# ANRGUSC/DEFER

Hardware: NVIDIA H100
Metric: inferences_per_sec (higher is better)
Workload: dtype bf16x3->f32

## Files before the change

### defer_b200/csrc/conv_umma.cu

```cuda
#include <cuda.h>
#include <string.h>

#include <type_traits>

#include <vector>

#include "common.cuh"
#include "conv_umma.cuh"

namespace defer {

static int env_int(const char* name, int dflt) {
  const char* v = getenv(name);
  return v ? atoi(v) : dflt;
}

namespace {

constexpr int BM = 128;
constexpr int BK = 64;
constexpr int CONS_THREADS = 256;
constexpr int NUM_THREADS = CONS_THREADS + 128;
constexpr int SMEM_CAP = 227 * 1024 - 256;
constexpr int CTL_BYTES = 256;
constexpr int MAX_STAGES = 8;
constexpr int MEGA_BN = 64;
constexpr int STG_COLS = 64;
constexpr int STG_BYTES = BM * STG_COLS * 4;

struct KParams {
  int n, ho, wo, cout;
  int tile_n, tile_h, tile_w, tiles_h, tiles_w;
  int flat;
  int m_total;
  int kh, kw, sh, sw, pad_t, pad_l;
  int cblocks;
  int k_blocks;
  int splits;
  int cluster;
  uint32_t flags;
  const float* scale;
  const float* shift;
  const void* res;
  void* y;
  float* partial;
  unsigned int* counters;
  size_t plane_out;
};

struct alignas(128) MegaOp {
  CUtensorMap tmx[2];
  CUtensorMap tmw[2];
  KParams p;
  int m_tiles, n_tiles;
  const float* stem_x;
  int stem_h, stem_w, stem_cin, stem_kh, stem_kw, stem_sh, stem_sw, stem_pad_t, stem_pad_l, stem_K;
  int stem_win_rows, stem_win_cols;
  const uint8_t* stem_u8;
  float stem_shift[3];
  const float* scale2;
  const float* shift2;
  void* y2;
  int relu2;
  int store_first;
};

template <int NPLANES, int BN>
struct Smem {
  static constexpr int A_PLANE = BM * 128;
  static constexpr int B_PLANE = BN * 128;
  static constexpr int STAGE = NPLANES * (A_PLANE + B_PLANE);
  static constexpr int RED = BM * BN * 4;
  __host__ __device__ static constexpr int ring(int stages, bool red) {
    return (red && stages * STAGE < RED) ? RED : stages * STAGE;
  }
  __host__ __device__ static constexpr int total(int stages, bool red) {
    return ring(stages, red) + STG_BYTES + CTL_BYTES + 1024;
  }
  __host__ __device__ static constexpr int max_stages() {
    return (SMEM_CAP - STG_BYTES - CTL_BYTES - 1024) / STAGE > MAX_STAGES ? MAX_STAGES
                                                                          : (SMEM_CAP - STG_BYTES - CTL_BYTES - 1024) / STAGE;
  }
};
static_assert(Smem<2, 128>::max_stages() == 3 && Smem<2, 64>::max_stages() == 4, "BF16X2 ring depths");
static_assert(Smem<1, 64>::max_stages() == 8 && Smem<1, 128>::max_stages() == 6, "BF16 ring depths");

__device__ __forceinline__ uint32_t smem_u32(const void* p) { return (uint32_t)__cvta_generic_to_shared(p); }

__device__ __forceinline__ void mbar_init(uint32_t bar, uint32_t count) {
  asm volatile("mbarrier.init.shared::cta.b64 [%0], %1;" ::"r"(bar), "r"(count));
}
__device__ __forceinline__ void mbar_arrive_expect_tx(uint32_t bar, uint32_t bytes) {
  asm volatile("mbarrier.arrive.expect_tx.shared::cta.b64 _, [%0], %1;" ::"r"(bar), "r"(bytes) : "memory");
}
__device__ __forceinline__ void mbar_expect_tx(uint32_t bar, uint32_t bytes) {
  asm volatile("mbarrier.expect_tx.relaxed.cta.shared::cta.b64 [%0], %1;" ::"r"(bar), "r"(bytes) : "memory");
}
__device__ __forceinline__ void mbar_arrive(uint32_t bar) {
  asm volatile("mbarrier.arrive.shared::cta.b64 _, [%0];" ::"r"(bar) : "memory");
}
__device__ __forceinline__ bool mbar_try_wait(uint32_t bar, uint32_t parity) {
  uint32_t ok;
  asm volatile(
      "{\n.reg .pred p;\n"
      "mbarrier.try_wait.parity.shared::cta.b64 p, [%1], %2;\n"
      "selp.u32 %0, 1, 0, p;\n}\n"
      : "=r"(ok)
      : "r"(bar), "r"(parity)
      : "memory");
  return ok != 0;
}
__device__ __forceinline__ unsigned long long gtimer() {
  unsigned long long t;
  asm volatile("mov.u64 %0, %%globaltimer;" : "=l"(t));
  return t;
}
__device__ int g_conv_wait_timeout_tag;
__device__ __forceinline__ void mbar_wait(uint32_t bar, uint32_t parity, int tag) {
  if (mbar_try_wait(bar, parity)) return;
  unsigned long long t0 = gtimer();
  unsigned spins = 0;
  while (!mbar_try_wait(bar, parity)) {
    if ((++spins & 0xfff) == 0 && gtimer() - t0 > 2000000000ull) {
      g_conv_wait_timeout_tag = tag;
      asm volatile("trap;");
    }
  }
}

__device__ __forceinline__ void tma_load_4d(uint32_t dst, const CUtensorMap* map, uint32_t bar, int c0, int c1, int c2,
                                            int c3) {
  asm volatile(
      "cp.async.bulk.tensor.4d.shared::cluster.global.mbarrier::complete_tx::bytes [%0], [%1, {%3, %4, %5, %6}], [%2];"
      ::"r"(dst), "l"(reinterpret_cast<uint64_t>(map)), "r"(bar), "r"(c0), "r"(c1), "r"(c2), "r"(c3)
      : "memory");
}
__device__ __forceinline__ void tma_load_3d(uint32_t dst, const CUtensorMap* map, uint32_t bar, int c0, int c1, int c2) {
  asm volatile(
      "cp.async.bulk.tensor.3d.shared::cluster.global.mbarrier::complete_tx::bytes [%0], [%1, {%3, %4, %5}], [%2];"
      ::"r"(dst), "l"(reinterpret_cast<uint64_t>(map)), "r"(bar), "r"(c0), "r"(c1), "r"(c2)
      : "memory");
}

__device__ __forceinline__ void cluster_sync_all() {
  asm volatile("barrier.cluster.arrive.release.aligned;" ::: "memory");
  asm volatile("barrier.cluster.wait.acquire.aligned;" ::: "memory");
}
__device__ __forceinline__ uint32_t cluster_ctarank() {
  uint32_t r;
  asm volatile("mov.u32 %0, %%cluster_ctarank;" : "=r"(r));
  return r;
}
__device__ __forceinline__ uint32_t cluster_nctarank() {
  uint32_t r;
  asm volatile("mov.u32 %0, %%cluster_nctarank;" : "=r"(r));
  return r;
}
__device__ __forceinline__ uint32_t dsmem_map(uint32_t local_addr, uint32_t rank) {
  uint32_t r;
  asm volatile("mapa.shared::cluster.u32 %0, %1, %2;" : "=r"(r) : "r"(local_addr), "r"(rank));
  return r;
}
__device__ __forceinline__ float4 dsmem_ld4(uint32_t addr) {
  float4 v;
  asm volatile("ld.shared::cluster.v4.f32 {%0, %1, %2, %3}, [%4];" : "=f"(v.x), "=f"(v.y), "=f"(v.z), "=f"(v.w) : "r"(addr));
  return v;
}
__device__ __forceinline__ void cons_bar_sync() { asm volatile("bar.sync 1, 256;" ::: "memory"); }
__device__ __forceinline__ void prod_bar_sync() { asm volatile("bar.sync 2, 128;" ::: "memory"); }

__device__ __forceinline__ uint64_t make_sw128_desc(uint32_t smem_addr) {
  return (uint64_t)((smem_addr & 0x3FFFF) >> 4) | (1ull << 16) | (64ull << 32) | (1ull << 62);
}
__device__ __forceinline__ void wg_fence() { asm volatile("wgmma.fence.sync.aligned;" ::: "memory"); }
__device__ __forceinline__ void wg_commit() { asm volatile("wgmma.commit_group.sync.aligned;" ::: "memory"); }
template <int N>
__device__ __forceinline__ void wg_wait() {
  asm volatile("wgmma.wait_group.sync.aligned %0;" ::"n"(N) : "memory");
}
template <int R>
__device__ __forceinline__ void acc_fence(float (&d)[R]) {
#pragma unroll
  for (int i = 0; i < R; ++i) asm volatile("" : "+f"(d[i])::"memory");
}

template <int BN>
__device__ __forceinline__ void wgmma_bf16(float (&d)[BN / 2], uint64_t a, uint64_t b);
// ... 244 lines not shown
  __shared__ int s_is_last;

  const int tid = threadIdx.x;
  if (tid == 0) {
    for (int s = 0; s < stages; ++s) {
      mbar_init(full_bar(s), 1);
      mbar_init(empty_bar(s), CONS_THREADS / 32);
    }
    asm volatile("fence.mbarrier_init.release.cluster;" ::: "memory");
  }
  __syncthreads();
  if (pdl) {
    asm volatile("griddepcontrol.wait;" ::: "memory");
    asm volatile("griddepcontrol.launch_dependents;" ::: "memory");
  }

  uint32_t it = 0;
  for (int o = 0; o < n_ops; ++o) {
    const MegaOp& op = ops[o];
    const KParams& p = op.p;
    const int total = op.m_tiles * op.n_tiles;
    int t_first, t_step;
    if (MODE == 0) {
      t_first = blockIdx.y * op.m_tiles + blockIdx.x;
      t_step = total;
    } else if (MODE == 1) {
      t_first = blockIdx.x;
      t_step = gridDim.x;
    } else {
      t_first = (int)cluster_ctarank();
      t_step = (int)cluster_nctarank();
    }
    const int split = MODE == 0 ? (int)blockIdx.z : 0;
    const int kb_begin = (split * p.k_blocks) / p.splits;
    const int kb_end = ((split + 1) * p.k_blocks) / p.splits;

    for (int t = t_first; t < total; t += t_step) {
      const int m_tile = t % op.m_tiles;
      const int c_base = (t / op.m_tiles) * BN;
      int n0 = 0, h0 = 0, w0 = 0;
      if (p.flat) {
        w0 = m_tile * BM;
      } else {
        const int tw = m_tile % p.tiles_w;
        const int t2 = m_tile / p.tiles_w;
        n0 = (t2 / p.tiles_h) * p.tile_n;
        h0 = (t2 % p.tiles_h) * p.tile_h;
        w0 = tw * p.tile_w;
      }

      if (tid >= CONS_THREADS) {
        if (tid == CONS_THREADS) {
          const uint32_t a_rows = p.flat ? (uint32_t)BM : (uint32_t)(p.tile_n * p.tile_h * p.tile_w);
          uint32_t i2 = it;
          for (int kb = kb_begin; kb < kb_end; ++kb, ++i2) {
            const int stage = (int)(i2 % (uint32_t)stages);
            const uint32_t phase = (i2 / (uint32_t)stages) & 1u;
            mbar_wait(empty_bar(stage), phase ^ 1u, 1);
            const uint32_t a_dst = ring + stage * L::STAGE;
            const uint32_t b_dst = a_dst + NPLANES * L::A_PLANE;
            const int tap = kb / p.cblocks;
            const int cb = kb - tap * p.cblocks;
            const int khi = tap / p.kw;
            const int kwi = tap - khi * p.kw;
            int cw = w0, ch = 0, cn = 0;
            if (!p.flat) {
              cw = w0 * p.sw + kwi - p.pad_l;
              ch = h0 * p.sh + khi - p.pad_t;
              cn = n0;
            }
            mbar_arrive_expect_tx(full_bar(stage), NPLANES * (a_rows * 128u + (uint32_t)L::B_PLANE));
            tma_load_4d(a_dst, &op.tmx[0], full_bar(stage), cb * BK, cw, ch, cn);
            tma_load_3d(b_dst, &op.tmw[0], full_bar(stage), cb * BK, c_base, tap);
            if (NPLANES == 2) {
              tma_load_4d(a_dst + L::A_PLANE, &op.tmx[1], full_bar(stage), cb * BK, cw, ch, cn);
              tma_load_3d(b_dst + L::B_PLANE, &op.tmw[1], full_bar(stage), cb * BK, c_base, tap);
            }
          }
        }
        it += (uint32_t)(kb_end - kb_begin);
        continue;
      }

      const int wg = tid >> 7;
      const int lane = tid & 31;
      float acc[R];
#pragma unroll
      for (int i = 0; i < R; ++i) acc[i] = 0.f;
      int prev_stage = -1;
      for (int kb = kb_begin; kb < kb_end; ++kb, ++it) {
        const int stage = (int)(it % (uint32_t)stages);
        mbar_wait(full_bar(stage), (it / (uint32_t)stages) & 1u, 2);
        const uint32_t a_addr = ring + stage * L::STAGE + wg * (64 * 128);
        const uint32_t b_addr = ring + stage * L::STAGE + NPLANES * L::A_PLANE;
        wg_fence();
#pragma unroll
        for (int k = 0; k < BK / 16; ++k) {
          const uint64_t a_hi = make_sw128_desc(a_addr + k * 32);
          const uint64_t b_hi = make_sw128_desc(b_addr + k * 32);
          wgmma_bf16<BN>(acc, a_hi, b_hi);
          if (NPLANES == 2) {
            wgmma_bf16<BN>(acc, make_sw128_desc(a_addr + L::A_PLANE + k * 32), b_hi);
            wgmma_bf16<BN>(acc, a_hi, make_sw128_desc(b_addr + L::B_PLANE + k * 32));
          }
        }
        wg_commit();
        wg_wait<1>();
        acc_fence(acc);
        if (prev_stage >= 0 && lane == 0) mbar_arrive(empty_bar(prev_stage));
        prev_stage = stage;
      }
      wg_wait<0>();
      acc_fence(acc);
      if (prev_stage >= 0 && lane == 0) mbar_arrive(empty_bar(prev_stage));


      if (MODE == 0 && p.cluster) {
        cons_bar_sync();
        float4* red_buf = reinterpret_cast<float4*>(smem);
#pragma unroll
        for (int q = 0; q < R / 4; ++q)
          red_buf[q * CONS_THREADS + tid] = make_float4(acc[4 * q], acc[4 * q + 1], acc[4 * q + 2], acc[4 * q + 3]);
        break;
      }
      if (MODE == 0 && p.splits > 1) {
        const size_t tile_lin = (size_t)t;
        float4* mine = reinterpret_cast<float4*>(p.partial) + (tile_lin * p.splits + split) * (R / 4) * CONS_THREADS;
#pragma unroll
        for (int q = 0; q < R / 4; ++q)
// ... 313 lines not shown
          wgmma_bf16<64>(acc, make_sw128_desc(a_addr + L::A_PLANE + k * 32), b_hi);
          wgmma_bf16<64>(acc, a_hi, make_sw128_desc(b_addr + L::B_PLANE + k * 32));
        }
      }
      wg_commit();
      wg_wait<1>();
      acc_fence(acc);
      if (prev_stage >= 0 && lane == 0) mbar_arrive(empty_bar(prev_stage));
      prev_stage = stage;
    }
    wg_wait<0>();
    acc_fence(acc);
    if (prev_stage >= 0 && lane == 0) mbar_arrive(empty_bar(prev_stage));
    int n0, h0, w0;
    stem_tile_origin(p, t % op.m_tiles, n0, h0, w0);
    epi_tile<NPLANES, 64, false>(p, epi_args(op), stg, acc, 0xffffu, (t / op.m_tiles) * 64, n0, h0, w0);
  }
}

template <int NPLANES>
__global__ void __launch_bounds__(NUM_THREADS, 1) conv_stem_kernel(const MegaOp* __restrict__ ops, int stages, int pdl) {
  stem_body<NPLANES, STEM_F32>(ops, stages, pdl);
}

template <int NPLANES>
__global__ void __launch_bounds__(NUM_THREADS, 1) conv_stem_u8_kernel(const MegaOp* __restrict__ ops, int stages, int pdl) {
  stem_body<NPLANES, STEM_U8_CAFFE>(ops, stages, pdl);
}

template <int NPLANES>
__global__ void __launch_bounds__(NUM_THREADS, 1) conv_stem_u8tf_kernel(const MegaOp* __restrict__ ops, int stages, int pdl) {
  stem_body<NPLANES, STEM_U8_TF>(ops, stages, pdl);
}

__global__ void __launch_bounds__(256) weight_transform_kernel(const float* __restrict__ w, __nv_bfloat16* __restrict__ out,
                                                               int taps, int cin, int cout, int nplanes) {
  size_t total = (size_t)taps * cin * cout;
  size_t i = (size_t)blockIdx.x * blockDim.x + threadIdx.x;
  if (i >= total) return;
  int ci = (int)(i % cin);
  size_t t2 = i / cin;
  int co = (int)(t2 % cout);
  int tap = (int)(t2 / cout);
  float v = w[((size_t)tap * cin + ci) * cout + co];
  __nv_bfloat16 hi = __float2bfloat16_rn(v);
  out[i] = hi;
  if (nplanes == 2) out[total + i] = __float2bfloat16_rn(v - __bfloat162float(hi));
}

typedef CUresult (*PFN_encodeTiled)(CUtensorMap*, CUtensorMapDataType, cuuint32_t, void*, const cuuint64_t*,
                                    const cuuint64_t*, const cuuint32_t*, const cuuint32_t*, CUtensorMapInterleave,
                                    CUtensorMapSwizzle, CUtensorMapL2promotion, CUtensorMapFloatOOBfill);

PFN_encodeTiled get_encode() {
  static PFN_encodeTiled fn = nullptr;
  if (!fn) {
    void* p = nullptr;
    cudaDriverEntryPointQueryResult q;
    if (cudaGetDriverEntryPoint("cuTensorMapEncodeTiled", &p, cudaEnableDefault, &q) == cudaSuccess &&
        q == cudaDriverEntryPointSuccess)
      fn = (PFN_encodeTiled)p;
  }
  return fn;
}

int encode_map(CUtensorMap* map, void* base, int rank, const uint64_t* dims, const uint64_t* strides_bytes,
               const uint32_t* box, const uint32_t* estr) {
  PFN_encodeTiled enc = get_encode();
  if (!enc) {
    set_error("cuTensorMapEncodeTiled entry point not available");
    return DEFER_ERR_CUDA;
  }
  CUresult r = enc(map, CU_TENSOR_MAP_DATA_TYPE_BFLOAT16, (cuuint32_t)rank, base, (const cuuint64_t*)dims,
                   (const cuuint64_t*)strides_bytes, (const cuuint32_t*)box, (const cuuint32_t*)estr,
                   CU_TENSOR_MAP_INTERLEAVE_NONE, CU_TENSOR_MAP_SWIZZLE_128B, CU_TENSOR_MAP_L2_PROMOTION_L2_256B,
                   CU_TENSOR_MAP_FLOAT_OOB_FILL_NONE);
  if (r != CUDA_SUCCESS) {
    set_error("cuTensorMapEncodeTiled failed (CUresult %d): rank %d dims [%llu,%llu,%llu,%llu] box [%u,%u,%u,%u]", (int)r,
              rank, (unsigned long long)dims[0], (unsigned long long)dims[1], (unsigned long long)(rank > 2 ? dims[2] : 0),
              (unsigned long long)(rank > 3 ? dims[3] : 0), box[0], box[1], rank > 2 ? box[2] : 0, rank > 3 ? box[3] : 0);
    return DEFER_ERR_CUDA;
  }
  return DEFER_OK;
}

template <auto kernel>
int set_smem_attr(bool cluster16 = false) {
  static bool attr_set[64] = {false};
  int dev = 0;
  DEFER_CUDA(cudaGetDevice(&dev));
  if (dev < 64 && !attr_set[dev]) {
    DEFER_CUDA(cudaFuncSetAttribute(kernel, cudaFuncAttributeMaxDynamicSharedMemorySize, SMEM_CAP));
    if (cluster16) DEFER_CUDA(cudaFuncSetAttribute(kernel, cudaFuncAttributeNonPortableClusterSizeAllowed, 1));
    prefer_max_smem(kernel);
    attr_set[dev] = true;
  }
  return DEFER_OK;
}

int sm_count() {
  static int sms[64] = {0};
  int dev = 0;
  if (cudaGetDevice(&dev) != cudaSuccess || dev >= 64) return 1;
  if (!sms[dev]) cudaDeviceGetAttribute(&sms[dev], cudaDevAttrMultiProcessorCount, dev);
  return sms[dev] > 0 ? sms[dev] : 1;
}

void fill_op(const UmmaConvPlan& P, const UmmaConvLaneArgs& a, MegaOp* out) {
  MegaOp& op = *out;
  memset(&op, 0, sizeof op);
  op.tmx[0] = a.tmap_x[0];
  op.tmx[1] = a.tmap_x[1];
  op.tmw[0] = P.tmap_w[0];
  op.tmw[1] = P.tmap_w[1];
  KParams& kp = op.p;
  kp.n = P.n; kp.ho = P.ho; kp.wo = P.wo; kp.cout = P.cout;
  kp.tile_n = P.tile_n; kp.tile_h = P.tile_h; kp.tile_w = P.tile_w; kp.tiles_h = P.tiles_h; kp.tiles_w = P.tiles_w;
  kp.flat = P.flat;
  kp.m_total = P.n * P.ho * P.wo;
  kp.kh = P.kh; kp.kw = P.kw; kp.sh = P.sh; kp.sw = P.sw; kp.pad_t = P.pad_t; kp.pad_l = P.pad_l;
  kp.cblocks = P.cin / 64;
  kp.k_blocks = P.k_blocks;
  kp.splits = P.splits;
  kp.cluster = P.cluster;
  kp.flags = P.flags;
  kp.scale = P.scale; kp.shift = P.shift;
  kp.res = (P.flags & DEFER_FLAG_RESIDUAL) ? a.res : nullptr;
  kp.y = a.y;
  kp.partial = a.partial;
  kp.counters = a.counters;
  kp.plane_out = (size_t)P.n * P.ho * P.wo * P.cout;
  op.m_tiles = P.tiles_n * P.tiles_h * P.tiles_w;
  op.n_tiles = P.cout / P.bn;
  op.scale2 = P.scale2;
  op.shift2 = P.shift2;
  op.y2 = a.y2;
  op.relu2 = P.relu2;
  op.store_first = P.aff ? P.store_first : 1;
}

template <int NPLANES, int BN, bool AFF = false>
int launch_op_t(const UmmaConvPlan& P, const UmmaConvLaneArgs& a, cudaStream_t st) {
  using L = Smem<NPLANES, BN>;
  constexpr auto kernel = AFF ? &conv_umma_aff_kernel<NPLANES, BN> : &conv_umma_kernel<NPLANES, BN>;
  DEFER_TRY((set_smem_attr<kernel>()));
  MegaOp op;
  fill_op(P, a, &op);
  int stages = P.stages < 2 ? 2 : (P.stages > L::max_stages() ? L::max_stages() : P.stages);
  const size_t smem = (size_t)L::total(stages, P.cluster != 0);
  dim3 grid(op.m_tiles, op.n_tiles, P.splits);
  static const int pdl = env_int("DEFER_PDL", 0);
  if (pdl || P.cluster) {
    cudaLaunchConfig_t cfg;
    memset(&cfg, 0, sizeof cfg);
    cfg.gridDim = grid;
    cfg.blockDim = dim3(NUM_THREADS, 1, 1);
    cfg.dynamicSmemBytes = smem;
    cfg.stream = st;
    cudaLaunchAttribute attr[2];
    int na = 0;
    if (pdl) {
      attr[na].id = cudaLaunchAttributeProgrammaticStreamSerialization;
      attr[na].val.programmaticStreamSerializationAllowed = 1;
      ++na;
    }
    if (P.cluster) {
      attr[na].id = cudaLaunchAttributeClusterDimension;
      attr[na].val.clusterDim.x = 1;
      attr[na].val.clusterDim.y = 1;
      attr[na].val.clusterDim.z = (unsigned)P.splits;
      ++na;
    }
    cfg.attrs = attr;
    cfg.numAttrs = na;
    DEFER_CUDA(cudaLaunchKernelEx(&cfg, kernel, op, stages, pdl));
    return DEFER_OK;
  }
  kernel<<<grid, NUM_THREADS, smem, st>>>(op, stages, 0);
  DEFER_CUDA(cudaGetLastError());
  return DEFER_OK;
}

template <auto kernel>
int launch_grid(const void* dev_op, int n_tiles, int stages, size_t smem, cudaStream_t st) {
  DEFER_TRY((set_smem_attr<kernel>()));
  const int sms = sm_count();
  int grid = sms < n_tiles ? sms : n_tiles;
  const int rounds = (n_tiles + grid - 1) / grid;
  grid = (n_tiles + rounds - 1) / rounds;
  static const int pdl = env_int("DEFER_PDL", 0);
  if (pdl) {
    cudaLaunchConfig_t cfg;
    memset(&cfg, 0, sizeof cfg);
    cfg.gridDim = dim3(grid, 1, 1);
    cfg.blockDim = dim3(NUM_THREADS, 1, 1);
    cfg.dynamicSmemBytes = smem;
    cfg.stream = st;
    cudaLaunchAttribute attr[1];
    attr[0].id = cudaLaunchAttributeProgrammaticStreamSerialization;
    attr[0].val.programmaticStreamSerializationAllowed = 1;
    cfg.attrs = attr;
    cfg.numAttrs = 1;
    DEFER_CUDA(cudaLaunchKernelEx(&cfg, kernel, reinterpret_cast<const MegaOp*>(dev_op), stages, 1));
    return DEFER_OK;
  }
  kernel<<<grid, NUM_THREADS, smem, st>>>(reinterpret_cast<const MegaOp*>(dev_op), stages, 0);
  DEFER_CUDA(cudaGetLastError());
  return DEFER_OK;
}

template <int NPLANES, int BN, bool AFF = false>
int launch_persist_t(const void* dev_op, int n_tiles, int stages, cudaStream_t st) {
  using L = Smem<NPLANES, BN>;
  constexpr auto kernel = AFF ? &conv_stream_aff_kernel<NPLANES, BN> : &conv_stream_kernel<NPLANES, BN>;
  if (stages > L::max_stages()) stages = L::max_stages();
  if (stages < 2) stages = 2;
  return launch_grid<kernel>(dev_op, n_tiles, stages, (size_t)L::total(stages, false), st);
}

template <int NPLANES, int IN>
int launch_stem_t(const void* dev_op, int n_tiles, int stages, cudaStream_t st) {
  using L = StemSmem<NPLANES>;
  constexpr auto kernel = IN == STEM_U8_TF      ? &conv_stem_u8tf_kernel<NPLANES>
                          : IN == STEM_U8_CAFFE ? &conv_stem_u8_kernel<NPLANES>
                                                : &conv_stem_kernel<NPLANES>;
  if (stages > L::max_stages()) stages = L::max_stages();
  if (stages < 2) stages = 2;
  return launch_grid<kernel>(dev_op, n_tiles, stages, (size_t)L::total(stages), st);
}

template <int NPLANES>
int launch_mega_t(const void* dev_ops, int n_ops, int stages, cudaStream_t st) {
  using L = Smem<NPLANES, MEGA_BN>;
  DEFER_TRY(set_smem_attr<conv_mega_kernel<NPLANES>>(true));
  if (stages < 2) stages = 2;
  if (stages > L::max_stages()) stages = L::max_stages();
  const int cluster = umma_mega_cluster_size();
  cudaLaunchConfig_t cfg;
  memset(&cfg, 0, sizeof cfg);
  cfg.gridDim = dim3(cluster, 1, 1);
  cfg.blockDim = dim3(NUM_THREADS, 1, 1);
  cfg.dynamicSmemBytes = L::total(stages, false);
  cfg.stream = st;
  cudaLaunchAttribute attr[1];
  attr[0].id = cudaLaunchAttributeClusterDimension;
  attr[0].val.clusterDim.x = cluster;
  attr[0].val.clusterDim.y = 1;
  attr[0].val.clusterDim.z = 1;
  cfg.attrs = attr;
  cfg.numAttrs = 1;
  DEFER_CUDA(cudaLaunchKernelEx(&cfg, conv_mega_kernel<NPLANES>, reinterpret_cast<const MegaOp*>(dev_ops), n_ops, stages));
  return DEFER_OK;
}

}

bool umma_conv_supported(int fmt, int n, int h, int w, int cin, int ho, int wo, int cout, int kh, int kw, int sh, int sw,
                         int pad_t, int pad_l) {
  if (fmt != FMT_BF16X2 && fmt != FMT_BF16) return false;
  if (cin % 64 != 0 || cout % 64 != 0) return false;
  if (sh < 1 || sw < 1 || sh > 2 || sw > 2) return false;
  if (kh > 7 || kw > 7) return false;
  if (n < 1 || ho < 1 || wo < 1 || h < 1 || w < 1) return false;
  if ((size_t)n * ho * wo * cout >= (1ull << 40)) return false;
  (void)pad_t; (void)pad_l;
  return true;
}

int umma_conv_prepare(UmmaConvPlan* plan, int fmt, int n, int h, int w, int cin, int ho, int wo, int cout, int kh, int kw,
                      int sh, int sw, int pad_t, int pad_l, uint32_t flags, const float* w_hwio_dev, const float* scale_dev,
                      const float* shift_dev, bool mega, int stream_bn) {
  UmmaConvPlan& P = *plan;
  P = UmmaConvPlan();
  P.fmt = fmt;
  P.nplanes = fmt == FMT_BF16X2 ? 2 : 1;
  P.n = n; P.h = h; P.w = w; P.cin = cin; P.ho = ho; P.wo = wo; P.cout = cout;
  P.kh = kh; P.kw = kw; P.sh = sh; P.sw = sw; P.pad_t = pad_t; P.pad_l = pad_l;
  P.flags = flags;
  P.scale = scale_dev;
  P.shift = shift_dev;
  const int taps = kh * kw;
  P.k_blocks = taps * (cin / 64);

  P.flat = (kh == 1 && kw == 1 && sh == 1 && sw == 1 && pad_t == 0 && pad_l == 0 && ho == h && wo == w) ? 1 : 0;
  if (P.flat) {
    long long m = (long long)n * ho * wo;
    P.tile_n = 1; P.tile_h = 1; P.tile_w = BM;
    P.tiles_n = 1; P.tiles_h = 1; P.tiles_w = (int)((m + BM - 1) / BM);
  } else {
    int parts_w = (wo + BM - 1) / BM;
    P.tile_w = (wo + parts_w - 1) / parts_w;
    P.tiles_w = (wo + P.tile_w - 1) / P.tile_w;
    P.tile_h = BM / P.tile_w;
    if (P.tile_h > ho) P.tile_h = ho;
    P.tiles_h = (ho + P.tile_h - 1) / P.tile_h;
    P.tile_h = (ho + P.tiles_h - 1) / P.tiles_h;
    P.tile_n = 1;
    if (P.tile_h == ho && P.tiles_w == 1) {
      P.tile_n = BM / (P.tile_h * P.tile_w);
      if (P.tile_n > n) P.tile_n = n;
      if (P.tile_n < 1) P.tile_n = 1;
    }
    P.tiles_n = (n + P.tile_n - 1) / P.tile_n;
    if (P.tile_w * sw > 256 || P.tile_h * sh > 256) {
      set_error("umma conv: TMA box too large (tile %dx%d stride %dx%d)", P.tile_h, P.tile_w, sh, sw);
      return DEFER_ERR_INVALID;
    }
  }
  const int m_tiles = P.tiles_n * P.tiles_h * P.tiles_w;

  P.bn = (cout % 128 == 0 && (long long)m_tiles * (cout / 128) >= env_int("DEFER_UMMA_BN128_MIN_CTAS", 1)) ? 128 : 64;
  int force_bn = env_int("DEFER_UMMA_BN", 0);
  if (force_bn == 64 || (force_bn == 128 && cout % 128 == 0)) P.bn = force_bn;
  int ctas = m_tiles * (cout / P.bn);
  P.splits = 1;
  int target = env_int("DEFER_UMMA_TARGET_CTAS", 4);
  if (env_int("DEFER_UMMA_SPLITK", 1) && ctas < target && P.k_blocks >= 8) {
    int s = (target + ctas - 1) / ctas;
    int max_s = P.k_blocks / 4;
    if (s > max_s) s = max_s;
    if (s > 16) s = 16;
    if (s < 1) s = 1;
    int per = (P.k_blocks + s - 1) / s;
    P.splits = (P.k_blocks + per - 1) / per;
  }
  int force_split = env_int("DEFER_UMMA_FORCE_SPLITS", 0);
  if (force_split > 0 && force_split <= P.k_blocks) {
    int per = (P.k_blocks + force_split - 1) / force_split;
    P.splits = (P.k_blocks + per - 1) / per;
  }
  P.cluster = 0;
  if (env_int("DEFER_UMMA_CLUSTER", 0) && force_split <= 0 && !mega) {
    const int min_kb = env_int("DEFER_UMMA_CSPLIT_KB", 4);
    int max_s = env_int("DEFER_UMMA_CSPLIT_MAX", 8);
    if (max_s > 8) max_s = 8;
    const int max_ctas = env_int("DEFER_UMMA_CSPLIT_MAX_CTAS", 256);
    int s = 1;
    for (int c = 2; c <= max_s; c *= 2)
      if (P.k_blocks / c >= min_kb && (long long)ctas * c <= max_ctas) s = c;
    int force_c = env_int("DEFER_UMMA_FORCE_CSPLIT", 0);
    if ((force_c == 2 || force_c == 4 || force_c == 8) && P.k_blocks >= force_c) s = force_c;
    P.splits = s;
    P.cluster = s > 1 ? 1 : 0;
  }
  if (mega) {
    P.bn = MEGA_BN;
    P.splits = 1;
    P.cluster = 0;
  }
  if (stream_bn > 0) {
    P.bn = (stream_bn == 128 && cout % 128 == 0) ? 128 : 64;
    P.splits = 1;
    P.cluster = 0;
    P.stream = 1;
  }
  {
    int kb_per = (P.k_blocks + P.splits - 1) / P.splits;
    int st = kb_per <= 2 ? 2 : (kb_per <= 6 ? 3 : 4);
    int force_st = env_int("DEFER_UMMA_STAGES", 0);
    if (force_st > 0) st = force_st;
    P.stages = st;
  }

  size_t welems = (size_t)taps * cin * cout;
  DEFER_CUDA(cudaMalloc(&P.w_dev, welems * 2 * P.nplanes));
  {
    unsigned grid = (unsigned)((welems + 255) / 256);
    prefer_max_smem(weight_transform_kernel);
    weight_transform_kernel<<<grid, 256>>>(w_hwio_dev, (__nv_bfloat16*)P.w_dev, taps, cin, cout, P.nplanes);
    DEFER_CUDA(cudaGetLastError());
  }
  for (int pl = 0; pl < P.nplanes; ++pl) {
    uint64_t dims[3] = {(uint64_t)cin, (uint64_t)cout, (uint64_t)taps};
    uint64_t strides[2] = {(uint64_t)cin * 2, (uint64_t)cin * cout * 2};
    uint32_t box[3] = {64, (uint32_t)P.bn, 1};
    uint32_t es[3] = {1, 1, 1};
    DEFER_TRY(encode_map(&P.tmap_w[pl], (uint8_t*)P.w_dev + pl * welems * 2, 3, dims, strides, box, es));
  }
  if (P.nplanes == 1) P.tmap_w[1] = P.tmap_w[0];
  P.ready = true;
  return DEFER_OK;
}

int umma_conv_bind(const UmmaConvPlan& P, UmmaConvLaneArgs* a, const void* x, const void* res, void* y) {
  if (!P.ready) {
    set_error("umma_conv_bind: plan not prepared");
    return DEFER_ERR_STATE;
  }
  size_t xelems = (size_t)P.n * P.h * P.w * P.cin;
  for (int pl = 0; pl < P.nplanes; ++pl) {
    uint8_t* base = (uint8_t*)x + pl * xelems * 2;
    if (P.flat) {
      uint64_t m = (uint64_t)P.n * P.h * P.w;
      uint64_t dims[4] = {(uint64_t)P.cin, m, 1, 1};
      uint64_t strides[3] = {(uint64_t)P.cin * 2, m * P.cin * 2, m * P.cin * 2};
      uint32_t box[4] = {64, BM, 1, 1};
      uint32_t es[4] = {1, 1, 1, 1};
      DEFER_TRY(encode_map(&a->tmap_x[pl], base, 4, dims, strides, box, es));
    } else {
      uint64_t dims[4] = {(uint64_t)P.cin, (uint64_t)P.w, (uint64_t)P.h, (uint64_t)P.n};
      uint64_t strides[3] = {(uint64_t)P.cin * 2, (uint64_t)P.w * P.cin * 2, (uint64_t)P.h * P.w * P.cin * 2};
      uint32_t box[4] = {64, (uint32_t)(P.tile_w * P.sw), (uint32_t)(P.tile_h * P.sh), (uint32_t)P.tile_n};
      uint32_t es[4] = {1, (uint32_t)P.sw, (uint32_t)P.sh, 1};
      DEFER_TRY(encode_map(&a->tmap_x[pl], base, 4, dims, strides, box, es));
    }
  }
  if (P.nplanes == 1) a->tmap_x[1] = a->tmap_x[0];
  a->res = res;
  a->y = y;
  a->partial = nullptr;
  a->counters = nullptr;
  if (P.splits > 1 && !P.cluster) {
    size_t tiles = (size_t)P.tiles_n * P.tiles_h * P.tiles_w * (P.cout / P.bn);
    DEFER_CUDA(cudaMalloc((void**)&a->partial, tiles * P.splits * BM * P.bn * sizeof(float)));
    DEFER_CUDA(cudaMalloc((void**)&a->counters, tiles * sizeof(unsigned int)));
    DEFER_CUDA(cudaMemset(a->counters, 0, tiles * sizeof(unsigned int)));
  }
  return DEFER_OK;
}

void umma_conv_unbind(UmmaConvLaneArgs* a) {
  if (a->partial) cudaFree(a->partial);
  if (a->counters) cudaFree(a->counters);
  a->partial = nullptr;
  a->counters = nullptr;
}

int launch_conv_umma(const UmmaConvPlan& P, const UmmaConvLaneArgs& a, cudaStream_t st) {
  if (P.aff) {
    if (P.nplanes == 2) return P.bn == 128 ? launch_op_t<2, 128, true>(P, a, st) : launch_op_t<2, 64, true>(P, a, st);
    return P.bn == 128 ? launch_op_t<1, 128, true>(P, a, st) : launch_op_t<1, 64, true>(P, a, st);
  }
  if (P.nplanes == 2) return P.bn == 128 ? launch_op_t<2, 128>(P, a, st) : launch_op_t<2, 64>(P, a, st);
  return P.bn == 128 ? launch_op_t<1, 128>(P, a, st) : launch_op_t<1, 64>(P, a, st);
}

size_t umma_mega_op_bytes() { return sizeof(MegaOp); }

int umma_mega_fill(void* host_dst, const UmmaConvPlan& P, const UmmaConvLaneArgs& a) {
  if (!P.ready || (P.bn != MEGA_BN && !P.stream) || P.splits != 1) {
    set_error("umma_mega_fill: plan is not a persistent-kernel plan (bn %d, splits %d)", P.bn, P.splits);
    return DEFER_ERR_STATE;
  }
  MegaOp op;
  fill_op(P, a, &op);
// ... 102 lines not shown
```

### defer_b200/csrc/conv_umma.cuh

```cuda
#pragma once
#include <cuda.h>
#include <cuda_runtime.h>
#include <stdint.h>

namespace defer {

struct UmmaConvPlan {
  int fmt = 0, nplanes = 1;
  int n = 0, h = 0, w = 0, cin = 0, ho = 0, wo = 0, cout = 0;
  int kh = 1, kw = 1, sh = 1, sw = 1, pad_t = 0, pad_l = 0;
  uint32_t flags = 0;
  int tile_n = 1, tile_h = 1, tile_w = 1, tiles_n = 1, tiles_h = 1, tiles_w = 1;
  int flat = 0;
  int bn = 64;
  int k_blocks = 0;
  int splits = 1;
  int cluster = 0;
  int stages = 4;
  int stream = 0;
  void* w_dev = nullptr;
  const float* scale = nullptr;
  const float* shift = nullptr;
  bool aff = false;
  const float* scale2 = nullptr;
  const float* shift2 = nullptr;
  int relu2 = 0;
  int store_first = 1;
  CUtensorMap tmap_w[2];
  bool ready = false;
};

struct UmmaConvLaneArgs {
  CUtensorMap tmap_x[2];
  bool direct_out = false;
  const void* res = nullptr;
  void* y = nullptr;
  void* y2 = nullptr;
  float* partial = nullptr;
  unsigned int* counters = nullptr;
};

bool umma_conv_supported(int fmt, int n, int h, int w, int cin, int ho, int wo, int cout, int kh, int kw, int sh, int sw,
                         int pad_t, int pad_l);
int umma_conv_prepare(UmmaConvPlan* plan, int fmt, int n, int h, int w, int cin, int ho, int wo, int cout, int kh, int kw,
                      int sh, int sw, int pad_t, int pad_l, uint32_t flags, const float* w_hwio_dev, const float* scale_dev,
                      const float* shift_dev, bool mega = false, int stream_bn = 0);
int umma_conv_bind(const UmmaConvPlan& plan, UmmaConvLaneArgs* args, const void* x, const void* res, void* y);
void umma_conv_unbind(UmmaConvLaneArgs* args);
int launch_conv_umma(const UmmaConvPlan& plan, const UmmaConvLaneArgs& args, cudaStream_t st);
void umma_conv_release(UmmaConvPlan& plan);

size_t umma_mega_op_bytes();
int umma_mega_fill(void* host_dst, const UmmaConvPlan& plan, const UmmaConvLaneArgs& args);
int umma_mega_cluster_size();
int launch_conv_mega(int nplanes, const void* dev_ops, int n_ops, cudaStream_t st);
int launch_conv_stream(int nplanes, int bn, const void* dev_op, int n_tiles, int k_blocks, bool aff, cudaStream_t st);
bool umma_stem_fusable(int fmt, int cin, int ho, int wo, int cout, int kh, int kw, int sh, int sw, uint32_t flags);
int umma_mega_set_stem(void* host_op, const float* x, int h, int w, int cin, int kh, int kw, int sh, int sw, int pad_t, int pad_l);
void umma_mega_set_stem_u8(void* host_op, const uint8_t* x, const float shift[3]);
int launch_conv_stem(int nplanes, const void* dev_op, int n_tiles, bool u8, bool tf, cudaStream_t st);
int launch_conv_persistent(int nplanes, const void* dev_op, int n_tiles, bool aff, cudaStream_t st);

}
```

### defer_b200/csrc/stage.cu

```cuda
#include <stdarg.h>
#include <string.h>
#include <unistd.h>

#include <mutex>
#include <set>
#include <utility>
#include <stdlib.h>
#include <string>
#include <vector>

#include "common.cuh"
#include "conv_umma.cuh"

namespace defer {

static thread_local char g_err[1024] = "";
void set_error(const char* fmt, ...) {
  va_list ap;
  va_start(ap, fmt);
  vsnprintf(g_err, sizeof(g_err), fmt, ap);
  va_end(ap);
}
const char* get_error() { return g_err; }

// ... 641 lines not shown
        return fail(DEFER_ERR_CUDA);
      }
    }
    if (cfg->is_last) {
      if (cudaMallocHost((void**)&L.out_host, s->bufs[cfg->output_buf].elems * 4) != cudaSuccess ||
          cudaMallocHost((void**)&L.status_host, sizeof(int)) != cudaSuccess) {
        set_error("cudaMallocHost result buffer failed");
        return fail(DEFER_ERR_CUDA);
      }
      *L.status_host = 0;
    }
    L.umma.resize(n_ops);
  }
  if (cudaDeviceSynchronize() != cudaSuccess) {
    set_error("device sync after stage setup failed: %s", cudaGetErrorString(cudaGetLastError()));
    return fail(DEFER_ERR_CUDA);
  }
  *out = s;
  return DEFER_OK;
}

int defer_stage_destroy(defer_stage_t s) {
  if (!s) return DEFER_OK;
  cudaSetDevice(s->cfg.device);
  cudaDeviceSynchronize();
  for (auto& L : s->lanes) {
    if (L.exec) cudaGraphExecDestroy(L.exec);
    if (L.graph) cudaGraphDestroy(L.graph);
    if (L.stream) cudaStreamDestroy(L.stream);
    if (L.done) cudaEventDestroy(L.done);
    if (L.join) cudaEventDestroy(L.join);
    if (L.t0) cudaEventDestroy(L.t0);
    if (L.t1) cudaEventDestroy(L.t1);
    for (auto& ua : L.umma) umma_conv_unbind(&ua);
    if (L.out_host) cudaFreeHost(L.out_host);
    if (L.status_host) cudaFreeHost(L.status_host);
  }
  for (auto& op : s->ops)
    if (op.backend == 2 || op.backend == 4) umma_conv_release(op.umma);
  for (void* p : s->workspace) cudaFree(p);
  for (void* p : s->d_weights) if (p) cudaFree(p);
  for (void* p : s->d_weights_bf16) if (p) cudaFree(p);
  if (s->cons_arena && s->cons_is_ipc) cudaIpcCloseMemHandle(s->cons_arena);
  if (s->prod_arena && s->prod_is_ipc) cudaIpcCloseMemHandle(s->prod_arena);
  for (auto& m : s->marks) if (m.ev) cudaEventDestroy(m.ev);
  if (s->job_t0) cudaEventDestroy(s->job_t0);
  if (s->job_t1) cudaEventDestroy(s->job_t1);
  if (s->flush_buf) cudaFree(s->flush_buf);
  if (s->arena) cudaFree(s->arena);
  delete s;
  return DEFER_OK;
}

int defer_stage_describe(defer_stage_t s, char* buf, size_t buf_len) {
  DEFER_CHECK(s && buf && buf_len > 0, "describe: null");
  std::string o;
  char line[512];
  static const char* fm[] = {"f32", "bf16x2", "bf16"};
  snprintf(line, sizeof line, "stage device=%d fmt=%s batch=%d depth=%d first=%d last=%d ops=%zu prod=%d cons=%d\n",
           s->cfg.device, fm[s->cfg.fmt], s->cfg.batch, s->cfg.depth, s->cfg.is_first, s->cfg.is_last, s->ops.size(),
           (int)s->has_prod, (int)s->has_cons);
  o += line;
  for (size_t i = 0; i < s->ops.size(); ++i) {
    const OpRt& op = s->ops[i];
    const Buf& bi = s->bufs[op.d.in0];
    const Buf& bo = s->bufs[op.d.out];
    if (!s->op_group.empty() && s->op_group[i] >= 0 && (int)i == s->groups[s->op_group[i]].first) {
      snprintf(line, sizeof line, "  -- megakernel group: ops %d..%d in one cluster launch --\n", s->groups[s->op_group[i]].first,
               s->groups[s->op_group[i]].last);
      o += line;
    }
    snprintf(line, sizeof line, "  [%2zu] %-22s in b%-3d(%d,%d,%d) res b%-3d -> b%-3d(%d,%d,%d) k=%dx%d s=%d flags=%u  %.3f MB %.3f GF\n", i,
             op.kname.c_str(), op.d.in0, bi.h, bi.w, bi.c, op.d.in1, op.d.out, bo.h, bo.w, bo.c, op.d.kh, op.d.kw, op.d.sh,
             op.d.flags, op.alg_bytes / 1e6, op.alg_flops / 1e9);
    o += line;
    if ((op.backend == 2 || op.backend == 4) && op.umma.ready) {
      const UmmaConvPlan& u = op.umma;
      snprintf(line, sizeof line, "       wgmma tiles: m=%d x n=%d (BN %d) x k-splits %d%s, %d k-blocks, ring %d -> %d CTAs\n",
               u.tiles_n * u.tiles_h * u.tiles_w, u.cout / u.bn, u.bn, u.splits, u.cluster ? " (cluster, DSMEM reduce)" : "",
               u.k_blocks, u.stages, u.tiles_n * u.tiles_h * u.tiles_w * (u.cout / u.bn) * u.splits);
      o += line;
    }
  }
  strncpy(buf, o.c_str(), buf_len - 1);
  buf[buf_len - 1] = 0;
  return DEFER_OK;
}

int defer_stage_io_bytes(defer_stage_t s, uint64_t* in_bytes, uint64_t* out_bytes) {
  DEFER_CHECK(s, "io_bytes: null");
  if (in_bytes) *in_bytes = s->bufs[s->cfg.input_buf].bytes;
  if (out_bytes) *out_bytes = s->bufs[s->cfg.output_buf].bytes;
  return DEFER_OK;
}

static int fill_token(defer_stage_t s, int role, LinkToken* t) {
  memset(t, 0, sizeof(*t));
  t->magic = TOKEN_MAGIC;
  t->role = role;
  t->device = s->cfg.device;
  t->pid = (int)getpid();
  t->depth = s->cfg.depth;
  t->fmt = s->cfg.fmt;
  t->batch = s->cfg.batch;
  t->slot_bytes = role == 0 ? s->bufs[s->cfg.input_buf].bytes : s->bufs[s->cfg.output_buf].bytes;
  t->arena_bytes = s->arena_bytes;
  t->off_slots = CTRL_BYTES;
  t->slot_stride = s->slot_stride;
  t->local_base = (uint64_t)(uintptr_t)s->arena;
  return DEFER_OK;
}

static int apply_token(defer_stage_t s, int role, const LinkToken* t, uint8_t* mapped, bool is_ipc) {
  DEFER_CHECK(t->depth == s->cfg.depth && t->fmt == s->cfg.fmt && t->batch == s->cfg.batch,
              "link: depth/fmt/batch mismatch (peer %d/%d/%d, mine %d/%d/%d)", t->depth, t->fmt, t->batch, s->cfg.depth,
              s->cfg.fmt, s->cfg.batch);
  if (role == 0) {
    DEFER_CHECK(!s->cfg.is_last, "link: the last stage has no consumer");
    DEFER_CHECK(t->slot_bytes == s->bufs[s->cfg.output_buf].bytes, "link: my output is %zu bytes, consumer slot is %llu",
                s->bufs[s->cfg.output_buf].bytes, (unsigned long long)t->slot_bytes);
    s->cons_arena = mapped;
    s->cons_is_ipc = is_ipc;
    s->cons_off_slots = t->off_slots;
    s->cons_slot_stride = t->slot_stride;
    for (int l = 0; l < s->cfg.depth; ++l) {
      void* slot = mapped + t->off_slots + t->slot_stride * l;
      if (s->hop == HOP_COPY) s->lanes[l].peer_out = slot;
      else s->lanes[l].buf[s->cfg.output_buf] = slot;
    }
    s->has_cons = true;
  } else {
    DEFER_CHECK(!s->cfg.is_first, "link: the first stage has no producer");
    DEFER_CHECK(t->slot_bytes == s->bufs[s->cfg.input_buf].bytes, "link: my input is %zu bytes, producer sends %llu",
// ... 586 lines not shown
```

Baseline: 14390.

## Load conv A tiles with TMA im2col mode for flat 128-row M tiling

Adds a TMA im2col tensor map path so non-1x1 convolutions can tile M as contiguous 128 output pixels (flat) instead of 4-D spatial boxes, with per-tap kernel offsets passed to the im2col copy. It is enabled by default when the padding corners fit the 8-bit offset range. The aim is full 128-row tiles with no waste from spatial boxes that do not align with the output shape. It also factors out the persistent grid computation and extends the describe output.

After: 15280 (median of 6 runs). +6.2%, better.

```diff
diff --git a/defer_b200/csrc/conv_umma.cu b/defer_b200/csrc/conv_umma.cu
--- a/defer_b200/csrc/conv_umma.cu
+++ b/defer_b200/csrc/conv_umma.cu
@@ -32,6 +32,7 @@
   int n, ho, wo, cout;
   int tile_n, tile_h, tile_w, tiles_h, tiles_w;
   int flat;
+  int im2col;
   int m_total;
   int kh, kw, sh, sw, pad_t, pad_l;
   int cblocks;
@@ -133,6 +134,14 @@
   asm volatile(
       "cp.async.bulk.tensor.4d.shared::cluster.global.mbarrier::complete_tx::bytes [%0], [%1, {%3, %4, %5, %6}], [%2];"
       ::"r"(dst), "l"(reinterpret_cast<uint64_t>(map)), "r"(bar), "r"(c0), "r"(c1), "r"(c2), "r"(c3)
+      : "memory");
+}
+__device__ __forceinline__ void tma_load_im2col_4d(uint32_t dst, const CUtensorMap* map, uint32_t bar, int c0, int c1, int c2,
+                                                   int c3, uint16_t ow, uint16_t oh) {
+  asm volatile(
+      "cp.async.bulk.tensor.4d.shared::cluster.global.im2col.mbarrier::complete_tx::bytes [%0], [%1, {%3, %4, %5, %6}], [%2], "
+      "{%7, %8};"
+      ::"r"(dst), "l"(reinterpret_cast<uint64_t>(map)), "r"(bar), "r"(c0), "r"(c1), "r"(c2), "r"(c3), "h"(ow), "h"(oh)
       : "memory");
 }
 __device__ __forceinline__ void tma_load_3d(uint32_t dst, const CUtensorMap* map, uint32_t bar, int c0, int c1, int c2) {
@@ -483,6 +492,14 @@
       if (tid >= CONS_THREADS) {
         if (tid == CONS_THREADS) {
           const uint32_t a_rows = p.flat ? (uint32_t)BM : (uint32_t)(p.tile_n * p.tile_h * p.tile_w);
+          int iw = 0, ih = 0, in_ = 0;
+          if (p.im2col) {
+            const int hw = p.ho * p.wo;
+            in_ = w0 / hw;
+            const int oh = (w0 - in_ * hw) / p.wo;
+            ih = oh * p.sh - p.pad_t;
+            iw = (w0 - in_ * hw - oh * p.wo) * p.sw - p.pad_l;
+          }
           uint32_t i2 = it;
           for (int kb = kb_begin; kb < kb_end; ++kb, ++i2) {
             const int stage = (int)(i2 % (uint32_t)stages);
@@ -501,11 +518,14 @@
               cn = n0;
             }
             mbar_arrive_expect_tx(full_bar(stage), NPLANES * (a_rows * 128u + (uint32_t)L::B_PLANE));
-            tma_load_4d(a_dst, &op.tmx[0], full_bar(stage), cb * BK, cw, ch, cn);
-            tma_load_3d(b_dst, &op.tmw[0], full_bar(stage), cb * BK, c_base, tap);
-            if (NPLANES == 2) {
-              tma_load_4d(a_dst + L::A_PLANE, &op.tmx[1], full_bar(stage), cb * BK, cw, ch, cn);
-              tma_load_3d(b_dst + L::B_PLANE, &op.tmw[1], full_bar(stage), cb * BK, c_base, tap);
+#pragma unroll
+            for (int pl = 0; pl < NPLANES; ++pl) {
+              if (p.im2col)
+                tma_load_im2col_4d(a_dst + pl * L::A_PLANE, &op.tmx[pl], full_bar(stage), cb * BK, iw, ih, in_, (uint16_t)kwi,
+                                   (uint16_t)khi);
+              else
+                tma_load_4d(a_dst + pl * L::A_PLANE, &op.tmx[pl], full_bar(stage), cb * BK, cw, ch, cn);
+              tma_load_3d(b_dst + pl * L::B_PLANE, &op.tmw[pl], full_bar(stage), cb * BK, c_base, tap);
             }
           }
         }
@@ -925,15 +945,27 @@
                                     const cuuint64_t*, const cuuint32_t*, const cuuint32_t*, CUtensorMapInterleave,
                                     CUtensorMapSwizzle, CUtensorMapL2promotion, CUtensorMapFloatOOBfill);
 
+typedef CUresult (*PFN_encodeIm2col)(CUtensorMap*, CUtensorMapDataType, cuuint32_t, void*, const cuuint64_t*,
+                                     const cuuint64_t*, const int*, const int*, cuuint32_t, cuuint32_t, const cuuint32_t*,
+                                     CUtensorMapInterleave, CUtensorMapSwizzle, CUtensorMapL2promotion,
+                                     CUtensorMapFloatOOBfill);
+
+void* driver_entry(const char* name) {
+  void* p = nullptr;
+  cudaDriverEntryPointQueryResult q;
+  if (cudaGetDriverEntryPoint(name, &p, cudaEnableDefault, &q) == cudaSuccess && q == cudaDriverEntryPointSuccess) return p;
+  return nullptr;
+}
+
 PFN_encodeTiled get_encode() {
   static PFN_encodeTiled fn = nullptr;
-  if (!fn) {
-    void* p = nullptr;
-    cudaDriverEntryPointQueryResult q;
-    if (cudaGetDriverEntryPoint("cuTensorMapEncodeTiled", &p, cudaEnableDefault, &q) == cudaSuccess &&
-        q == cudaDriverEntryPointSuccess)
-      fn = (PFN_encodeTiled)p;
-  }
+  if (!fn) fn = (PFN_encodeTiled)driver_entry("cuTensorMapEncodeTiled");
+  return fn;
+}
+
+PFN_encodeIm2col get_encode_im2col() {
+  static PFN_encodeIm2col fn = nullptr;
+  if (!fn) fn = (PFN_encodeIm2col)driver_entry("cuTensorMapEncodeIm2col");
   return fn;
 }
 
@@ -952,6 +984,43 @@
     set_error("cuTensorMapEncodeTiled failed (CUresult %d): rank %d dims [%llu,%llu,%llu,%llu] box [%u,%u,%u,%u]", (int)r,
               rank, (unsigned long long)dims[0], (unsigned long long)dims[1], (unsigned long long)(rank > 2 ? dims[2] : 0),
               (unsigned long long)(rank > 3 ? dims[3] : 0), box[0], box[1], rank > 2 ? box[2] : 0, rank > 3 ? box[3] : 0);
+    return DEFER_ERR_CUDA;
+  }
+  return DEFER_OK;
+}
+
+void im2col_corners(const UmmaConvPlan& P, int lower[2], int upper[2]) {
+  lower[0] = -P.pad_l;
+  lower[1] = -P.pad_t;
+  upper[0] = (P.wo - 1) * P.sw - P.pad_l - (P.w - 1);
+  upper[1] = (P.ho - 1) * P.sh - P.pad_t - (P.h - 1);
+}
+
+bool im2col_fits(const UmmaConvPlan& P) {
+  int lo[2], up[2];
+  im2col_corners(P, lo, up);
+  for (int d = 0; d < 2; ++d)
+    if (lo[d] < -128 || lo[d] > 127 || up[d] < -128 || up[d] > 127) return false;
+  return true;
+}
+
+int encode_im2col_map(CUtensorMap* map, void* base, const UmmaConvPlan& P) {
+  PFN_encodeIm2col enc = get_encode_im2col();
+  if (!enc) {
+    set_error("cuTensorMapEncodeIm2col entry point not available");
+    return DEFER_ERR_CUDA;
+  }
+  const uint64_t dims[4] = {(uint64_t)P.cin, (uint64_t)P.w, (uint64_t)P.h, (uint64_t)P.n};
+  const uint64_t strides[3] = {(uint64_t)P.cin * 2, (uint64_t)P.w * P.cin * 2, (uint64_t)P.h * P.w * P.cin * 2};
+  const uint32_t es[4] = {1, (uint32_t)P.sw, (uint32_t)P.sh, 1};
+  int lo[2], up[2];
+  im2col_corners(P, lo, up);
+  CUresult r = enc(map, CU_TENSOR_MAP_DATA_TYPE_BFLOAT16, 4, base, (const cuuint64_t*)dims, (const cuuint64_t*)strides, lo,
+                   up, (cuuint32_t)BK, (cuuint32_t)BM, (const cuuint32_t*)es, CU_TENSOR_MAP_INTERLEAVE_NONE,
+                   CU_TENSOR_MAP_SWIZZLE_128B, CU_TENSOR_MAP_L2_PROMOTION_L2_256B, CU_TENSOR_MAP_FLOAT_OOB_FILL_NONE);
+  if (r != CUDA_SUCCESS) {
+    set_error("cuTensorMapEncodeIm2col failed (CUresult %d): dims [%d,%d,%d,%d] corners (%d,%d)..(%d,%d) strides %dx%d",
+              (int)r, P.cin, P.w, P.h, P.n, lo[0], lo[1], up[0], up[1], P.sw, P.sh);
     return DEFER_ERR_CUDA;
   }
   return DEFER_OK;
@@ -989,7 +1058,8 @@
   KParams& kp = op.p;
   kp.n = P.n; kp.ho = P.ho; kp.wo = P.wo; kp.cout = P.cout;
   kp.tile_n = P.tile_n; kp.tile_h = P.tile_h; kp.tile_w = P.tile_w; kp.tiles_h = P.tiles_h; kp.tiles_w = P.tiles_w;
-  kp.flat = P.flat;
+  kp.flat = P.flat || P.im2col;
+  kp.im2col = P.im2col;
   kp.m_total = P.n * P.ho * P.wo;
   kp.kh = P.kh; kp.kw = P.kw; kp.sh = P.sh; kp.sw = P.sw; kp.pad_t = P.pad_t; kp.pad_l = P.pad_l;
   kp.cblocks = P.cin / 64;
@@ -1057,10 +1127,7 @@
 template <auto kernel>
 int launch_grid(const void* dev_op, int n_tiles, int stages, size_t smem, cudaStream_t st) {
   DEFER_TRY((set_smem_attr<kernel>()));
-  const int sms = sm_count();
-  int grid = sms < n_tiles ? sms : n_tiles;
-  const int rounds = (n_tiles + grid - 1) / grid;
-  grid = (n_tiles + rounds - 1) / rounds;
+  const int grid = umma_persistent_grid(n_tiles);
   static const int pdl = env_int("DEFER_PDL", 0);
   if (pdl) {
     cudaLaunchConfig_t cfg;
@@ -1128,6 +1195,13 @@
 
 }
 
+int umma_persistent_grid(int n_tiles) {
+  const int sms = sm_count();
+  const int grid = sms < n_tiles ? sms : n_tiles;
+  const int rounds = (n_tiles + grid - 1) / grid;
+  return (n_tiles + rounds - 1) / rounds;
+}
+
 bool umma_conv_supported(int fmt, int n, int h, int w, int cin, int ho, int wo, int cout, int kh, int kw, int sh, int sw,
                          int pad_t, int pad_l) {
   if (fmt != FMT_BF16X2 && fmt != FMT_BF16) return false;
@@ -1156,7 +1230,8 @@
   P.k_blocks = taps * (cin / 64);
 
   P.flat = (kh == 1 && kw == 1 && sh == 1 && sw == 1 && pad_t == 0 && pad_l == 0 && ho == h && wo == w) ? 1 : 0;
-  if (P.flat) {
+  P.im2col = (!P.flat && env_int("DEFER_IM2COL", 1) && im2col_fits(P)) ? 1 : 0;
+  if (P.flat || P.im2col) {
     long long m = (long long)n * ho * wo;
     P.tile_n = 1; P.tile_h = 1; P.tile_w = BM;
     P.tiles_n = 1; P.tiles_h = 1; P.tiles_w = (int)((m + BM - 1) / BM);
@@ -1263,7 +1338,9 @@
   size_t xelems = (size_t)P.n * P.h * P.w * P.cin;
   for (int pl = 0; pl < P.nplanes; ++pl) {
     uint8_t* base = (uint8_t*)x + pl * xelems * 2;
-    if (P.flat) {
+    if (P.im2col) {
+      DEFER_TRY(encode_im2col_map(&a->tmap_x[pl], base, P));
+    } else if (P.flat) {
       uint64_t m = (uint64_t)P.n * P.h * P.w;
       uint64_t dims[4] = {(uint64_t)P.cin, m, 1, 1};
       uint64_t strides[3] = {(uint64_t)P.cin * 2, m * P.cin * 2, m * P.cin * 2};
diff --git a/defer_b200/csrc/conv_umma.cuh b/defer_b200/csrc/conv_umma.cuh
--- a/defer_b200/csrc/conv_umma.cuh
+++ b/defer_b200/csrc/conv_umma.cuh
@@ -12,6 +12,7 @@
   uint32_t flags = 0;
   int tile_n = 1, tile_h = 1, tile_w = 1, tiles_n = 1, tiles_h = 1, tiles_w = 1;
   int flat = 0;
+  int im2col = 0;
   int bn = 64;
   int k_blocks = 0;
   int splits = 1;
@@ -55,6 +56,7 @@
 int umma_mega_cluster_size();
 int launch_conv_mega(int nplanes, const void* dev_ops, int n_ops, cudaStream_t st);
 int launch_conv_stream(int nplanes, int bn, const void* dev_op, int n_tiles, int k_blocks, bool aff, cudaStream_t st);
+int umma_persistent_grid(int n_tiles);
 bool umma_stem_fusable(int fmt, int cin, int ho, int wo, int cout, int kh, int kw, int sh, int sw, uint32_t flags);
 int umma_mega_set_stem(void* host_op, const float* x, int h, int w, int cin, int kh, int kw, int sh, int sw, int pad_t, int pad_l);
 void umma_mega_set_stem_u8(void* host_op, const uint8_t* x, const float shift[3]);
diff --git a/defer_b200/csrc/stage.cu b/defer_b200/csrc/stage.cu
--- a/defer_b200/csrc/stage.cu
+++ b/defer_b200/csrc/stage.cu
@@ -717,6 +717,8 @@
   return DEFER_OK;
 }
 
+static const char* tiling_name(const UmmaConvPlan& u) { return u.flat ? "flat" : (u.im2col ? "im2col" : "4-D box"); }
+
 int defer_stage_describe(defer_stage_t s, char* buf, size_t buf_len) {
   DEFER_CHECK(s && buf && buf_len > 0, "describe: null");
   std::string o;
@@ -741,9 +743,13 @@
     o += line;
     if ((op.backend == 2 || op.backend == 4) && op.umma.ready) {
       const UmmaConvPlan& u = op.umma;
-      snprintf(line, sizeof line, "       wgmma tiles: m=%d x n=%d (BN %d) x k-splits %d%s, %d k-blocks, ring %d -> %d CTAs\n",
+      const int tiles = u.tiles_n * u.tiles_h * u.tiles_w * (u.cout / u.bn);
+      char grid[32] = "";
+      if (op.persist && !op.stem_fused) snprintf(grid, sizeof grid, ", grid %d", umma_persistent_grid(tiles));
+      snprintf(line, sizeof line,
+               "       wgmma tiles: m=%d x n=%d (BN %d) x k-splits %d%s, %d k-blocks, ring %d -> %d CTAs, A %s%s\n",
                u.tiles_n * u.tiles_h * u.tiles_w, u.cout / u.bn, u.bn, u.splits, u.cluster ? " (cluster, DSMEM reduce)" : "",
-               u.k_blocks, u.stages, u.tiles_n * u.tiles_h * u.tiles_w * (u.cout / u.bn) * u.splits);
+               u.k_blocks, u.stages, tiles * u.splits, tiling_name(u), grid);
       o += line;
     }
   }
```
